# santi-pdp/segan_pytorch

Hardware: AMD Instinct MI355X
Metric: 16384-sample waveform chunks/sec (GAN step) (higher is better)
Workload: dtype f32

## Files before the change

segan_pytorch_amd/_lib.py:

```python
import ctypes
import os
import re
from ctypes import POINTER, Structure, c_char_p, c_double, c_float, c_int, c_int32, c_int64, c_size_t, c_void_p

_HERE = os.path.dirname(os.path.abspath(__file__))
LIB_PATH = os.environ.get('SEGAN_HIP_LIB') or os.path.join(_HERE, 'libsegan_hip.so')
HEADER_PATH = os.path.join(os.path.dirname(_HERE), 'include', 'segan_hip.h')
EXT_HEADER_PATH = os.path.join(os.path.dirname(_HERE), 'include', 'segan_dereverb.h')
PYIN_HEADER_PATH = os.path.join(os.path.dirname(_HERE), 'include', 'segan_pyin.h')
OMLSA_HEADER_PATH = os.path.join(os.path.dirname(_HERE), 'include', 'segan_omlsa.h')
RIR_HEADER_PATH = os.path.join(os.path.dirname(_HERE), 'include', 'segan_rir.h')


class SeganSrc(Structure):
    _fields_ = [('p0', c_void_p), ('p1', c_void_p), ('C0', c_int32), ('C1', c_int32),
                ('scale', c_void_p), ('shift', c_void_p), ('slope', c_void_p)]


_SCALARS = {'int': c_int, 'float': c_float, 'double': c_double, 'size_t': c_size_t,
            'int64_t': c_int64, 'long long': c_int64}


class _Defines(dict):

    def __init__(self, where):
        dict.__init__(self)
        self.where, self.unread = where, {}

    def __missing__(self, name):
        raise RuntimeError('{}: no integer `#define {}` ({})'.format(
            self.where, name, self.unread.get(name, 'not defined')))


def _ctype(text, decl, ret=False):
    tok = [w for w in re.findall(r'\w+|\S', text) if w != 'const']
    if not ret:
        if len(tok) < 2 or not re.match(r'[A-Za-z_]\w*$', tok[-1]):
            raise RuntimeError('unnamed or unreadable argument `{}` in `{}`'.format(text.strip(), decl))
        tok.pop()
    stars = tok.count('*')
    base = tok[:len(tok) - stars]
    if stars and base and '*' not in base:
        if not ret:
            return POINTER(SeganSrc) if tok == ['segan_src', '*'] else c_void_p
# ... 12 lines not shown
    seen = {}
    for name, val in re.findall(r'^[ \t]*#[ \t]*define[ \t]+(SEGAN_\w+)[ \t]+(\S.*?)[ \t]*$', text, flags=re.M):
        seen.setdefault(name, []).append(val)
    for name, vals in seen.items():
        if len(set(vals)) == 1 and re.match(r'-?(0[xX][0-9a-fA-F]+|[1-9]\d*|0)$', vals[0]):
            defines[name] = int(vals[0], 0)
        else:
            defines.unread[name] = ' / '.join('#define {} {}'.format(name, v) for v in vals)
    text = re.sub(r'^[ \t]*#.*$', '', text, flags=re.M)
    signatures = {}
    for m in re.finditer(r'[^;{}]*\bsegan_\w+\s*\([^;]*(;|$)', text):
        decl = ' '.join(m.group().split())
        d = re.match(r'([\w\s*]+?)\s*\b(segan_\w+)\s*\(([^()]*)\)\s*;$', decl)
        if not d or d.group(2) in signatures:
            raise RuntimeError('{}: cannot read the declaration `{}`'.format(where, decl))
        args = [] if d.group(3).strip() == 'void' else d.group(3).split(',')
        signatures[d.group(2)] = (_ctype(d.group(1), decl, ret=True), [_ctype(a, decl) for a in args])
    return signatures, defines


def _read_header_file(path=HEADER_PATH):
    if not os.path.exists(path):
        raise RuntimeError('segan_pytorch_amd: {} not found. The ctypes binding is read from the '
                           'header the library is built against.'.format(path))
    with open(path) as f:
        return read_header(f.read(), path)


SIGNATURES, DEFINES = _read_header_file()
EXT_SIGNATURES, EXT_DEFINES = _read_header_file(EXT_HEADER_PATH)
PYIN_SIGNATURES, PYIN_DEFINES = _read_header_file(PYIN_HEADER_PATH)
OMLSA_SIGNATURES, OMLSA_DEFINES = _read_header_file(OMLSA_HEADER_PATH)
RIR_SIGNATURES, RIR_DEFINES = _read_header_file(RIR_HEADER_PATH)

PAD_REFLECT = DEFINES['SEGAN_PAD_REFLECT']
PAD_ZERO = DEFINES['SEGAN_PAD_ZERO']
ACT_NONE = DEFINES['SEGAN_ACT_NONE']
ACT_TANH = DEFINES['SEGAN_ACT_TANH']
ABI_VERSION = DEFINES['SEGAN_ABI_VERSION']

_lib = None


def load():
    global _lib
    if _lib is not None:
        return _lib
    if not os.path.exists(LIB_PATH):
        raise RuntimeError(
            'segan_pytorch_amd: {} not found. Build it with `make` (or '
            '`python -c "import __graft_entry__ as g; g.build()"`) at the repo root. '
            'There is no non-HIP fallback.'.format(LIB_PATH))
    try:
        import torch
        if torch.cuda.is_available():
            torch.cuda.init()
    except ImportError:
        pass
    lib = ctypes.CDLL(LIB_PATH)
    for name, (res, args) in (list(SIGNATURES.items()) + list(EXT_SIGNATURES.items()) +
                              list(PYIN_SIGNATURES.items()) + list(OMLSA_SIGNATURES.items()) +
                              list(RIR_SIGNATURES.items())):
        fn = getattr(lib, name)
        fn.restype = res
        fn.argtypes = args
    ver = lib.segan_abi_version()
    if ver != ABI_VERSION:
        raise RuntimeError('libsegan_hip ABI {} != expected {}'.format(ver, ABI_VERSION))
    _lib = lib
    return lib


def check(rc, what=''):
    if rc != 0:
        msg = load().segan_last_error()
        raise RuntimeError('libsegan_hip {} failed ({}): {}'.format(
            what, rc, msg.decode() if msg else '?'))
```

segan_pytorch_amd/csrc/segan_conv.hip:

```cpp
#include "segan_conv_tile.h"


struct TileWork {
  int tile, c0, c1;
  bool partial;
  int piece;
};

struct TileIter {
  int tileA;
  long unit, unit_end;
  int first_tile;
  __device__ __forceinline__ void init(const CorrArgs& a, int nch) {
    tileA = blockIdx.x;
    unit = (long)blockIdx.x * a.sk_units;
    unit_end = min(unit + (long)a.sk_units, a.sk_total);
    first_tile = (int)(unit / nch);
  }
  __device__ __forceinline__ bool next(const CorrArgs& a, int nch, TileWork& w) {
    if (tileA < a.sk_nfull) {
      const int rd = tileA / (int)gridDim.x;
      const int left = a.sk_nfull - rd * (int)gridDim.x;
      w.tile = rd * (int)gridDim.x + xcd_remap(blockIdx.x, left < (int)gridDim.x ? left : (int)gridDim.x);
      w.c0 = 0; w.c1 = nch; w.partial = false; w.piece = 0;
      tileA += gridDim.x;
      return true;
    }
    if (unit < unit_end) {
      const int t = (int)(unit / nch);
      w.c0 = (int)(unit - (long)t * nch);
      w.c1 = min(nch, w.c0 + (int)(unit_end - unit));
      unit += w.c1 - w.c0;
      w.tile = a.sk_nfull + t;
// ... 890 lines not shown
  a.sk_ws_floats = scratch ? scratch_bytes / sizeof(float) : 0;
}

extern "C" size_t segan_bf16_scratch_bytes(int op, int B, int N, int M, int L, int K, int S, int pad,
                                           int planes) {
  if (!stride_ok(S) || B <= 0 || N <= 0 || M <= 0 || L <= 0 || L % S != 0 || planes < 1 || planes > 3)
    return 0;
  const int U = 32 / S, Ls = L / S;
  const size_t slabs = 256 + (size_t)1024 * 2 * 128 * 128 * sizeof(float);
  switch (op) {
    case 0: return slabs + segan_corr_bf2_scratch_bytes(B, N * S, Ls, U - 1, planes);
    case 3: return slabs + segan_corr_bf2_scratch_bytes(B, N * S, Ls, U - 1, planes);
    case 2: {
      int cmin = 1 << 30, cmax = 0;
      for (int r = 0; r < S; ++r) {
        const int c = (r + pad) / S;
        cmin = c < cmin ? c : cmin;
        cmax = c > cmax ? c : cmax;
      }
      return slabs + segan_corr_bf2_scratch_bytes(B, M, Ls, U - 1 + (cmax - cmin), planes);
    }
    case 1: {
      const int padR = K - S - pad > 0 ? K - S - pad : 0;
      return slabs + segan_corr_bf2_scratch_bytes(B, M, (L + pad + padR - 1) / S + 1, U - 1, planes);
    }
  }
  return 0;
}

extern "C" size_t segan_corr_scratch_bytes(void) {
  return (size_t)1024 * 2 * 128 * 128 * sizeof(float);
}

extern "C" int segan_conv1d_fwd(const segan_src* x, const void* wf, const float* bias, float* out,
                                int B, int N, int M, int L, int K, int S, int padL, int mode,
                                int roll, int precision, void* scratch, size_t scratch_bytes,
                                void* stream) {
  const int acc_block = precision == SEGAN_PREC_FP32_BLOCKED;
  if (acc_block) precision = SEGAN_PREC_FP32;
  SEGAN_REQUIRE(precision_ok(precision), "conv1d_fwd: precision must be 0, 1, 3 or 4");
  SEGAN_REQUIRE(stride_ok(S), "conv1d_fwd: stride %d not in {1,2,4}", S);
  SEGAN_REQUIRE(K >= 1 && K <= 32, "conv1d_fwd: kernel width %d not in [1,32]", K);
  SEGAN_REQUIRE(B > 0 && N > 0 && M > 0 && L > 0, "conv1d_fwd: bad sizes");
  SEGAN_REQUIRE(L % S == 0, "conv1d_fwd: length %d not divisible by stride %d", L, S);
  SEGAN_REQUIRE(wf && out, "conv1d_fwd: NULL pointer");
  SEGAN_REQUIRE(mode == SEGAN_PAD_REFLECT || mode == SEGAN_PAD_ZERO, "conv1d_fwd: bad pad mode");
  SEGAN_REQUIRE(mode != SEGAN_PAD_REFLECT || (padL < L && K - S - padL < L),
                "conv1d_fwd: reflect padding %d needs length > pad (L=%d)", padL, L);
  SEGAN_REQUIRE(roll > -L && roll < L, "conv1d_fwd: |roll| must be < L");
  if (int e = check_src(x, N, "conv1d_fwd")) return e;
  const int U = 32 / S;
  CorrArgs a = {};
  a.acc_block = acc_block;
  a.in = *x;
  a.wp = (const float*)wf;
  a.out0 = out; a.out1 = nullptr; a.bias = bias; a.halo = nullptr;
  a.B = B; a.Cv = N * S; a.Ktot = N * 32; a.RP = f_pitch(M); a.Rvalid = M;
  a.Tcols = L / S; a.Ctot = B * a.Tcols;
  a.Lin = L; a.padL = padL; a.mode = mode; a.roll = roll;
  a.win_start = 0; a.H = U - 1;
  a.NP = 1; a.Nout = 0;
  a.OC0 = M; a.OC1 = 0; a.Lout = a.Tcols; a.act = SEGAN_ACT_NONE;
  a.out0_elems = (size_t)B * M * a.Tcols;
  a.f_pair = f_pair(N, K); a.zphase = -1;
  if (precision) {
    CorrArgs a2 = a;
    const int e = segan_corr_bf2_f(a2, U, wf, precision, scratch, scratch_bytes, (hipStream_t)stream);
    return e;
  }
  if (N <= 2) return segan_launch_fsmall(a, M, N, S, (hipStream_t)stream);
  set_scratch(a, scratch, scratch_bytes);
  return launch_corr<true, false>(a, U, (hipStream_t)stream);
}

extern "C" int segan_deconv1d_dgrad(const float* dy, const void* wf, float* dx0, float* dx1, int B,
                                    int M, int M0, int N, int Ls, int K, int S, int pad,
                                    int precision, void* scratch, size_t scratch_bytes,
                                    void* stream) {
  const int acc_block = precision == SEGAN_PREC_FP32_BLOCKED;
  if (acc_block) precision = SEGAN_PREC_FP32;
  SEGAN_REQUIRE(precision_ok(precision), "deconv1d_dgrad: precision must be 0, 1, 3 or 4");
  SEGAN_REQUIRE(stride_ok(S), "deconv1d_dgrad: stride %d not in {1,2,4}", S);
  SEGAN_REQUIRE(K >= 1 && K <= 32, "deconv1d_dgrad: kernel width %d not in [1,32]", K);
  SEGAN_REQUIRE(B > 0 && N > 0 && M > 0 && Ls > 0, "deconv1d_dgrad: bad sizes");
  SEGAN_REQUIRE(M0 >= 0 && M0 <= M, "deconv1d_dgrad: split %d outside [0,%d]", M0, M);
  SEGAN_REQUIRE(dy && wf, "deconv1d_dgrad: NULL pointer");
  SEGAN_REQUIRE(dx0 || dx1, "deconv1d_dgrad: both destinations NULL");
  const int U = 32 / S;
  CorrArgs a = {};
  a.acc_block = acc_block;
  a.in.p0 = dy; a.in.p1 = nullptr; a.in.C0 = N; a.in.C1 = 0;
  a.in.scale = a.in.shift = a.in.slope = nullptr;
  a.wp = (const float*)wf;
  a.bias = nullptr; a.halo = nullptr;
  a.B = B; a.Cv = N * S; a.Ktot = N * 32; a.RP = f_pitch(M); a.Rvalid = M;
  a.Tcols = Ls; a.Ctot = B * Ls;
  a.Lin = S * Ls; a.padL = pad; a.mode = SEGAN_PAD_ZERO; a.roll = 0;
  a.win_start = 0; a.H = U - 1;
  a.NP = 1; a.Nout = 0;
  if (M0 == 0) { a.out0 = dx1; a.OC0 = M; a.out1 = nullptr; a.OC1 = 0; }
  else { a.out0 = dx0; a.OC0 = M0; a.out1 = dx1; a.OC1 = M - M0; }
  a.Lout = Ls; a.act = SEGAN_ACT_NONE;
  a.out0_elems = (size_t)B * a.OC0 * Ls;
  a.out1_elems = (size_t)B * a.OC1 * Ls;
  a.f_pair = f_pair(N, K); a.zphase = -1;
// ... 174 lines not shown
```

segan_pytorch_amd/csrc/segan_conv_edge.hip:

```cpp
#include "segan_conv_shared.h"

template <int S, int N, int PM, int KT>
__global__ __launch_bounds__(256) void tsmall_kernel(const CorrArgs a, const float* __restrict__ w,
                                                     int Krt, int M) {
  const int K = KT ? KT : Krt;
  constexpr int U = 32 / S;
  constexpr int MC = 16;
  constexpr int TW = 256 + U;
  __shared__ float xs[MC][TW + 1];
  const int tid = threadIdx.x;
  const int b = blockIdx.y;
  const int q0 = blockIdx.x * 256;
  const int q = q0 + tid;
  float acc[S][N];
#pragma unroll
  for (int r = 0; r < S; ++r)
#pragma unroll
    for (int n = 0; n < N; ++n) acc[r][n] = 0.0f;

  const int t0 = q0 + a.win_start + tid, t1 = t0 + 256;
  const bool ok0 = t0 >= 0 && t0 < a.Lin, ok1 = tid < U && t1 >= 0 && t1 < a.Lin;
  const int o0 = ok0 ? t0 : 0, o1 = ok1 ? t1 : 0;
  const int bo0 = b * a.in.C0 * a.Lin, bo1 = b * a.in.C1 * a.Lin;
  float pv0[MC], pv1[MC];
// ... 350 lines not shown
    float xv[N][32];
#pragma unroll
    for (int n = 0; n < N; ++n) {
      if (S == 4) {
#pragma unroll
        for (int i = 0; i < 8; ++i) {
          const f32x4 v = *reinterpret_cast<const f32x4*>(&xs[n][4 * tid + 4 * i]);
          xv[n][4 * i] = v[0]; xv[n][4 * i + 1] = v[1]; xv[n][4 * i + 2] = v[2]; xv[n][4 * i + 3] = v[3];
        }
      } else {
#pragma unroll
        for (int k = 0; k < 32; ++k) xv[n][k] = xs[n][S * tid + k];
      }
    }
    const int mcn = min(64, M - m0);
    for (int ml = 0; ml < mcn; ++ml) {
      float acc = a.bias ? a.bias[m0 + ml] : 0.0f;
#pragma unroll
      for (int n = 0; n < N; ++n) {
#pragma unroll
        for (int i = 0; i < 8; ++i) {
          const f32x4 wv = *reinterpret_cast<const f32x4*>(&ws[ml * WST + n * 32 + 4 * i]);
#pragma unroll
          for (int e = 0; e < 4; ++e) acc = fmaf(wv[e], xv[n][4 * i + e], acc);
        }
      }
      if (t < a.Lout) a.out0[((size_t)b * M + m0 + ml) * a.Lout + t] = acc;
    }
    __syncthreads();
  }
}


template <int S, int N, int RPT>
__global__ __launch_bounds__(256) void fsmall4_kernel(const CorrArgs a, const float* __restrict__ wq,
                                                      const float* __restrict__ bias, int M) {
  static_assert(S == 2 || S == 4, "fsmall4: strides 2 and 4");
  constexpr int Q = 4, U = 32 / S, MC = 8, CP = MC / 2;
  constexpr int XW = S * Q * 256 + 32;
  constexpr int XR = (S * (Q - 1) + 32 + 3) / 4 * 4;
  typedef float f32x2 __attribute__((ext_vector_type(2)));
  __shared__ __attribute__((aligned(16))) float xs[N][XW];
  const int tid = threadIdx.x;
  const int b = blockIdx.y;
  const int t0 = blockIdx.x * (Q * 256);
  fsmall_stage_window<S, N, XW>(a, b, t0, tid, xs);
  __syncthreads();
  const int t = t0 + Q * tid;
  f32x2 xv[N][XR / 2];
#pragma unroll
  for (int n = 0; n < N; ++n)
#pragma unroll
    for (int i = 0; i < XR / 4; ++i) {
      const f32x4 v = *reinterpret_cast<const f32x4*>(&xs[n][S * Q * tid + 4 * i]);
      xv[n][2 * i] = f32x2{v[0], v[1]};
      xv[n][2 * i + 1] = f32x2{v[2], v[3]};
    }
  const int RP = RPT ? RPT : a.RP;
  const bool vec = (a.Lout & 3) == 0 && t + Q <= a.Lout;
  typedef const __attribute__((address_space(4))) f32x2 cf2;
  for (int m0 = 0; m0 < M; m0 += MC) {
    f32x2 acc[CP][Q];
#pragma unroll
    for (int c = 0; c < CP; ++c) {
      const int ma = m0 + 2 * c < M ? m0 + 2 * c : M - 1, mb = m0 + 2 * c + 1 < M ? m0 + 2 * c + 1 : M - 1;
      const f32x2 bs = bias ? f32x2{bias[ma], bias[mb]} : f32x2{0.0f, 0.0f};
#pragma unroll
// ... 11 lines not shown
      }
    };
    auto fm = [&](const f32x2 (&w)[4][CP], int g, int e0, int e1) {
      const int n = g >> 3;
#pragma unroll
      for (int e = e0; e < e1; ++e)
#pragma unroll
        for (int c = 0; c < CP; ++c)
#pragma unroll
          for (int q = 0; q < Q; ++q) {
            const int j = S * q + 4 * (g & 7) + e;
            if (j & 1)
              asm("v_pk_fma_f32 %0, %1, %2, %0 op_sel:[0,1,0]"
                  : "+v"(acc[c][q]) : "s"(w[e][c]), "v"(xv[n][j >> 1]));
            else
              asm("v_pk_fma_f32 %0, %1, %2, %0 op_sel_hi:[1,0,1]"
                  : "+v"(acc[c][q]) : "s"(w[e][c]), "v"(xv[n][j >> 1]));
          }
    };
    ld(wa, 0);
#pragma unroll
    for (int g = 0; g < 8 * N; g += 2) {
      fm(wa, g, 0, 1);
      __builtin_amdgcn_sched_barrier(0);
      ld(wb, g + 1);
      __builtin_amdgcn_sched_barrier(0);
      fm(wa, g, 1, 4);
      fm(wb, g + 1, 0, 1);
      __builtin_amdgcn_sched_barrier(0);
      if (g + 2 < 8 * N) ld(wa, g + 2);
      __builtin_amdgcn_sched_barrier(0);
      fm(wb, g + 1, 1, 4);
    }
#pragma unroll
    for (int c = 0; c < MC; ++c) {
      if (m0 + c >= M) break;
      float* o = a.out0 + ((size_t)b * M + m0 + c) * a.Lout + t;
      if (vec) {
        const f32x4 ov = {acc[c / 2][0][c & 1], acc[c / 2][1][c & 1], acc[c / 2][2][c & 1], acc[c / 2][3][c & 1]};
        *reinterpret_cast<f32x4*>(o) = ov;
      } else {
#pragma unroll
        for (int q = 0; q < Q; ++q)
          if (t + q < a.Lout) o[q] = acc[c / 2][q][c & 1];
      }
    }
  }
}

int segan_launch_fsmall(CorrArgs& a, int M, int N, int S, hipStream_t st) {
  if (int e = segan_src_defaults(&a.in, st, "fsmall")) return e;
  if ((S == 4 || S == 2) && a.Lout >= 1024) {
    dim3 grid4(ceil_div(a.Lout, 1024), a.B);
#define FS4(SS, NN, RR) hipLaunchKernelGGL((fsmall4_kernel<SS, NN, RR>), grid4, dim3(256), 0, st, a, a.wp, a.bias, M)
    if (S == 4) {
      if (a.RP == 64) { if (N == 1) FS4(4, 1, 64); else FS4(4, 2, 64); }
      else { if (N == 1) FS4(4, 1, 0); else FS4(4, 2, 0); }
    } else {
      if (a.RP == 64) { if (N == 1) FS4(2, 1, 64); else FS4(2, 2, 64); }
      else { if (N == 1) FS4(2, 1, 0); else FS4(2, 2, 0); }
    }
#undef FS4
    return segan_check_launch("fsmall4_kernel");
  }
  dim3 grid(ceil_div(a.Lout, 256), a.B);
#define FS(SS, NN) hipLaunchKernelGGL((fsmall_kernel<SS, NN>), grid, dim3(256), 0, st, a, M)
  if (N == 1) { if (S == 4) FS(4, 1); else if (S == 2) FS(2, 1); else FS(1, 1); }
  else { if (S == 4) FS(4, 2); else if (S == 2) FS(2, 2); else FS(1, 2); }
#undef FS
  return segan_check_launch("fsmall_kernel");
}
```

segan_pytorch_amd/csrc/segan_conv_shared.h:

```cpp
#pragma once
#include "segan_common.h"
#include <stdlib.h>

#define KCH 64

struct ColTile {
  int col0, b0, t_first, len0;
};

__device__ __forceinline__ ColTile make_coltile(int col0, int Tcols, int NBcols) {
  ColTile t;
  t.col0 = col0;
  t.b0 = col0 / Tcols;
  t.t_first = col0 - t.b0 * Tcols;
  t.len0 = min(Tcols - t.t_first, NBcols);
  return t;
}

__device__ __forceinline__ void lds_pos_decode(const ColTile& ct, int j, int Tcols, int H, int& s,
                                               int& tau) {
  if (j < ct.len0 + H) {
    s = 0;
    tau = ct.t_first + j;
  } else {
// ... 11 lines not shown
  return x * q + (x < r ? x : r) + k;
}

struct CorrArgs {
  segan_src in;
  const float* wp;
  float* out0;
  float* out1;
  const float* bias;
  float* halo;
  int B, Cv, Ktot, RP, Rvalid;
  int Tcols, Ctot, ncoltiles;
  int Lin;
  int padL, mode, roll;
  int win_start, H, RLs;
  int rowshift[4];
  int NP, Nout;
  int OC0, OC1, Lout, act;
  int o_padL, o_roll, o_padR;
  int in_identity;
  int sk_nfull;
  int sk_units;
  long sk_total;
  int rt0;
  size_t out0_elems, out1_elems, halo_elems;
  float* sk_ws;
  size_t sk_ws_floats;
  int xf_mode;
  int acc_block;
  int RLv, nld;
  int f_pair;
  int zphase;
  int tile_order, nrt;
};



static inline int samples_per_tile(int Tcols, int NB) {
  if (Tcols >= NB) return (Tcols % NB == 0) ? 1 : 2;
  return (NB % Tcols == 0) ? NB / Tcols : (NB + Tcols - 2) / Tcols + 1;
}

static inline int t_np(int N, int S) { return round_up(N, 128 / S); }

struct WgradArgs {
  segan_src lo;
  segan_src hi;
  float* dw;
  int B, M, N, K, Ls, Lhi;
  int Cv;
  int padL, mode, roll;
  int Ctot;
  int cols_per_split;
  int H, RLw;
  int ls_magic;
  int per_magic;
  int bf_qc;
  int bf_cps;
  int Mp;
  int w2_cps, w2_nch;
  int w2_cpsample;
  int w2_spc;
  int w2_lsshift;
  int w2_pw, w2_nld;
  float* w2_slabs;
};
// ... 36 lines not shown
    int nb = 0;
    if (hipOccupancyMaxActiveBlocksPerMultiprocessor(&nb, reinterpret_cast<const void*>(kern), 256,
                                                     lds) != hipSuccess || nb < 1)
      nb = fallback;
    occ[d] = nb > 4 ? 4 : nb;
    occ_lds[d] = lds;
  }
  return occ[d];
}

static inline int f_pitch(int M) { return M <= 64 ? 64 : round_up(M, 128); }
static inline int f_rows(int N) { return round_up(N * 32, KCH); }
static inline int t_pitch(int N, int S) { return S * t_np(N, S); }
static inline int t_rows(int M, int S) { return round_up(M * (32 / S), KCH); }

static inline int f_pair(int N, int K) { return K == 31 && N > 2 && (N & 1) == 0; }
static inline int t_zphase(int K, int S, int pad_t) {
  return (K == 31 && S > 1) ? (((S - 1 - pad_t) % S) + S) % S : -1;
}

static inline bool stride_ok(int S) { return S == 1 || S == 2 || S == 4; }
static inline bool precision_ok(int p) { return p == 0 || p == 1 || p == 3; }
static inline int check_src(const segan_src* s, int C, const char* what) {
  SEGAN_REQUIRE(s != nullptr && s->p0 != nullptr, "%s: source is NULL", what);
  SEGAN_REQUIRE(s->C0 > 0 && s->C1 >= 0 && s->C0 + s->C1 == C,
                "%s: channel segments %d+%d != %d", what, s->C0, s->C1, C);
  SEGAN_REQUIRE(s->C1 == 0 || s->p1 != nullptr, "%s: second segment pointer is NULL", what);
  return SEGAN_OK;
}

int segan_launch_tsmall(CorrArgs& a, const float* w, int K, int M, int N, int S, int pad, hipStream_t st);
int segan_launch_fsmall(CorrArgs& a, int M, int N, int S, hipStream_t st);

void segan_note_corr_launch(int kind, unsigned grid, const CorrArgs& a, int ntiles);
int segan_corr_bf2_f(CorrArgs& a, int U, const void* wp3, int planes, void* scratch,
                     size_t scratch_bytes, hipStream_t st);
int segan_corr_bf2_t(CorrArgs& a, int U, const void* wp3, int planes, void* scratch,
                     size_t scratch_bytes, hipStream_t st);
size_t segan_corr_bf2_scratch_bytes(int B, int Cv, int Tcols, int H, int planes);
int segan_wgrad_bf2(WgradArgs& a, int U, int planes, void* scratch, size_t scratch_bytes, hipStream_t st);
void segan_note_wgrad_launch(int kind, int tiles, int nsplit, int chunks_per_split);
size_t segan_wgrad_bf2_scratch_bytes(int B, int M, int N, int Ls, int S, int planes);
```

segan_pytorch_amd/csrc/segan_pointwise.hip:

```cpp
#include "segan_common.h"

#define PW_THREADS 256

static int pw_nsplit(int B, int C, int L) {
  int ns = ceil_div(2048, C);
  if (ns > B) ns = B;
  long per = (long)B * L / ns;
  while (ns > 1 && per < 2048) {
    ns = (ns + 1) / 2;
    per = (long)B * L / ns;
  }
  return ns < 1 ? 1 : ns;
}

extern "C" int segan_bn_nsplit(int B, int C, int L) {
  if (B <= 0 || C <= 0 || L <= 0) return 0;
  return pw_nsplit(B, C, L);
}

template <int NV>
__device__ __forceinline__ void block_sum(float (&v)[NV], float* sm) {
  const int lane = threadIdx.x & 63, wave = threadIdx.x >> 6;
#pragma unroll
  for (int k = 0; k < NV; ++k) v[k] = warp_sum(v[k]);
  if (lane == 0)
#pragma unroll
    for (int k = 0; k < NV; ++k) sm[wave * NV + k] = v[k];
  __syncthreads();
  if (threadIdx.x == 0) {
#pragma unroll
    for (int k = 0; k < NV; ++k) {
      float s = 0.f;
      for (int w = 0; w < PW_THREADS / 64; ++w) s += sm[w * NV + k];
// ... 64 lines not shown
    }
  }
  float mean = 0.0f, m2 = 0.0f;
  if (n > 0.0f) {
    const float r = s1 / n;
    mean = K + r;
    m2 = fmaxf(s2 - s1 * r, 0.0f);
  }
#pragma unroll
  for (int o = 32; o > 0; o >>= 1) {
    const float nb2 = __shfl_down(n, o, 64), mb2 = __shfl_down(mean, o, 64), qb2 = __shfl_down(m2, o, 64);
    chan_combine(n, mean, m2, nb2, mb2, qb2);
  }
  const int lane = threadIdx.x & 63, wave = threadIdx.x >> 6;
  if (lane == 0) {
    sm[3 * wave] = n; sm[3 * wave + 1] = mean; sm[3 * wave + 2] = m2;
  }
  __syncthreads();
  if (threadIdx.x == 0) {
    for (int w = 1; w < PW_THREADS / 64; ++w) chan_combine(n, mean, m2, sm[3 * w], sm[3 * w + 1], sm[3 * w + 2]);
    float* w = ws + ((size_t)blockIdx.y * C + cr.c) * 3;
    w[0] = n;
    w[1] = mean;
    w[2] = m2;
  }
}

__device__ __forceinline__ void bn_affine(float gamma, float beta, float mean, float rstd,
                                          float& scale, float& shift) {
  scale = gamma * rstd;
  shift = fmaf(-mean, scale, beta);
}

__global__ void bn_final_kernel(const float* __restrict__ ws, const float* gamma, const float* beta,
                                float eps, float momentum, float* running_mean, float* running_var,
                                float* mean_o, float* rstd_o, float* scale_o, float* shift_o, int C,
                                int nsplit) {
  const int c = blockIdx.x * blockDim.x + threadIdx.x;
  if (c >= C) return;
  double n = 0.0, mean = 0.0, m2 = 0.0;
  for (int s = 0; s < nsplit; ++s) {
    const float* w = ws + ((size_t)s * C + c) * 3;
    const double nb = w[0], mb = w[1], qb = w[2];
    if (nb <= 0.0) continue;
    const double tot = n + nb;
    const double d = mb - mean;
    mean += d * nb / tot;
    m2 += qb + d * d * n * nb / tot;
    n = tot;
  }
  const double var = n > 0 ? m2 / n : 0.0;
  const float rstd = (float)(1.0 / sqrt(var + (double)eps));
  const float g = gamma ? gamma[c] : 1.0f;
  const float bt = beta ? beta[c] : 0.0f;
  float sc, sh;
  bn_affine(g, bt, (float)mean, rstd, sc, sh);
  if (mean_o) mean_o[c] = (float)mean;
  if (rstd_o) rstd_o[c] = rstd;
  if (scale_o) scale_o[c] = sc;
  if (shift_o) shift_o[c] = sh;
  if (running_mean) running_mean[c] = (1.0f - momentum) * running_mean[c] + momentum * (float)mean;
  if (running_var) {
    const double unb = n > 1 ? m2 / (n - 1.0) : var;
    running_var[c] = (1.0f - momentum) * running_var[c] + momentum * (float)unb;
  }
}

extern "C" int segan_bn_stats(const float* x, const float* gamma, const float* beta, float eps,
                              float momentum, float* running_mean, float* running_var, float* mean,
                              float* rstd, float* scale, float* shift, float* ws, int B, int C,
                              int L, void* stream) {
  SEGAN_REQUIRE(x && ws, "bn_stats: NULL pointer");
  SEGAN_REQUIRE(B > 0 && C > 0 && L > 0, "bn_stats: bad sizes");
  hipStream_t st = (hipStream_t)stream;
  const int ns = pw_nsplit(B, C, L);
  hipLaunchKernelGGL(bn_partial_kernel, dim3(C, ns), dim3(PW_THREADS), 0, st, x, ws, B, C, L, ns);
  hipLaunchKernelGGL(bn_final_kernel, dim3(ceil_div(C, 64)), dim3(64), 0, st, ws, gamma, beta, eps,
                     momentum, running_mean, running_var, mean, rstd, scale, shift, C, ns);
  return segan_check_launch("bn_stats");
}

extern "C" int segan_bn_partial(const float* x, float* ws, int B, int C, int L, void* stream) {
  SEGAN_REQUIRE(x && ws, "bn_partial: NULL pointer");
  SEGAN_REQUIRE(B > 0 && C > 0 && L > 0, "bn_partial: bad sizes");
  const int ns = pw_nsplit(B, C, L);
  hipLaunchKernelGGL(bn_partial_kernel, dim3(C, ns), dim3(PW_THREADS), 0, (hipStream_t)stream, x, ws,
                     B, C, L, ns);
  return segan_check_launch("bn_partial");
}

extern "C" int segan_bn_final(const float* ws, int nsplit_total, const float* gamma,
                              const float* beta, float eps, float momentum, float* running_mean,
                              float* running_var, float* mean, float* rstd, float* scale,
                              float* shift, int C, void* stream) {
  SEGAN_REQUIRE(ws && nsplit_total > 0 && C > 0, "bn_final: bad arguments");
  hipLaunchKernelGGL(bn_final_kernel, dim3(ceil_div(C, 64)), dim3(64), 0, (hipStream_t)stream, ws,
                     gamma, beta, eps, momentum, running_mean, running_var, mean, rstd, scale, shift,
                     C, nsplit_total);
// ... 721 lines not shown
```

segan_pytorch_amd/functional.py:

```python
import os

import torch

from . import ops
from .ops import ACT_NONE, ACT_TANH, PAD_REFLECT, PAD_ZERO, Src


def grad_buf(p):
    if p.grad is None:
        p.grad = torch.zeros_like(p, memory_format=torch.contiguous_format)
    elif not p.grad.is_contiguous():
        p.grad = p.grad.contiguous()
    return p.grad


def _gb(p, needed=True):
    if p is None or not needed or not p.requires_grad:
        return None
    return grad_buf(p)


def _bn_batch_stats(bn, training):
    return training or bn.running_mean is None or bn.running_var is None


def _bn_train_stats(c, bn, training=True):
    from . import distributed as sdist
    fn = sdist.bn_stats_sync if sdist.sync_bn_enabled() else ops.bn_stats
    track = training and bn.running_mean is not None and bn.running_var is not None
    momentum = 0.0
    if track:
        if bn.num_batches_tracked is not None:
            bn.num_batches_tracked += 1
        if bn.momentum is not None:
            momentum = bn.momentum
        else:
            momentum = 1.0 / float(bn.num_batches_tracked) if bn.num_batches_tracked is not None else 0.0
    return fn(c, bn.weight, bn.bias, bn.eps, momentum, bn.running_mean if track else None,
              bn.running_var if track else None)


def _bn_eval_affine(bn):
    rstd = torch.rsqrt(bn.running_var + bn.eps)
    gamma = bn.weight.detach() if bn.weight is not None else torch.ones_like(rstd)
    beta = bn.bias.detach() if bn.bias is not None else torch.zeros_like(rstd)
    scale = (gamma * rstd).contiguous()
    shift = (beta - bn.running_mean * scale).contiguous()
    return scale, shift, rstd.contiguous()


def _eval_bn_act_bwd(c, bn, scale, shift, rstd, dh, slope, dslope, y_tanh=None, dbias=None):
    if y_tanh is not None:
        g = ops.tanh_bwd(y_tanh, dh, dbias=_gb(bn.bias))
    else:
        v = ops.affine_prelu(c, scale, shift, None)
        g = ops.act_bwd(v, dh, slope=slope, dslope=dslope, dbias=_gb(bn.bias))
    if bn.weight is not None and bn.weight.requires_grad:
        xhat = ops.affine_prelu(c, rstd, (-bn.running_mean * rstd).contiguous(), None)
        grad_buf(bn.weight).add_((g * xhat).sum((0, 2)))
    dc = ops.affine_prelu(g, scale, None, None)
    if dbias is not None:
        ops.act_bwd(dc, dc, dbias=dbias)
    return dc


def _act_bwd_bn(a, dh, slope, bn, dslope, dgamma, dbeta, dbias):
    from . import distributed as sdist
    if sdist.sync_bn_enabled():
        return sdist.act_bwd_bn_sync(a, dh, slope, bn, dslope, dgamma, dbeta, dbias)
    return ops.act_bwd(a, dh, slope=slope, bn=bn, dslope=dslope, dgamma=dgamma, dbeta=dbeta,
                       dbias=dbias)

# ... 399 lines not shown
                if a_norm is None:
                    a_norm = ops.affine_prelu(a_enc[l], sc, sh, None)
                g = ops.act_bwd(a_norm, dh, dskip=dsk, slope=blk.act.weight, alpha=alpha_v,
                                dslope=_gb(blk.act.weight), dalpha=_gb(alpha_p, True))
                da = _act_bwd_bn(a_enc[l], g, None, bnsv, None, _gb(bnm.weight), _gb(bnm.bias),
                                 _gb(blk.conv.bias))
            padL = ops.conv_pad(K, S)[0]
            with _SideStream(da, src_enc[l]):
                if W.needs_grad(blk.conv):
                    gw = W.grad_target(blk.conv)
                    ops.wgrad(Src(da), src_enc[l], gw, K, S, padL, PAD_REFLECT)
                    W.finish(blk.conv, gw)
                _ready(blk, ready_extra)
            if l > 0:
                dh = ops.conv1d_dgrad(da, w, src_enc[l].L, S, pack=blk._pack)
            elif ctx.x_needs:
                dx = ops.conv1d_dgrad(da, w, src_enc[l].L, S, pack=blk._pack)
        _join_side(dy)
        ctx.state = None
        return (None, None, dx, None) + (None,) * (len(ctx.needs_input_grad) - 4)


class DiscriminatorFn(torch.autograd.Function):

    @staticmethod
    def forward(ctx, disc, rolls, x, x1, *params):
        x = x.contiguous()
        blocks = list(disc.enc_blocks)
        training = disc.training
        src = Src(x) if x1 is None else Src(x, x1.contiguous())
        cs, srcs, bns, xfs = [], [], [], []
        W = _Weights()
        for l, blk in enumerate(blocks):
            c = ops.conv1d_fwd(src, W.get(blk.conv), blk.conv.bias, blk.stride, roll=rolls[l],
                               pack=blk._pack)
            srcs.append(src)
            cs.append(c)
            if blk.norm is not None:
                bn = blk.norm
                if _bn_batch_stats(bn, training):
                    mean, rstd, scale, shift = _bn_train_stats(c, bn, training)
                    bns.append((mean, rstd, bn.weight, bn.bias))
                else:
                    scale, shift, _rstd = _bn_eval_affine(bn)
                    bns.append('eval')
                xfs.append((scale, shift))
                src = Src(c, scale=scale, shift=shift, slope=blk.act.weight)
            else:
                bns.append(None)
                xfs.append((None, None))
                src = Src(c, slope=blk.act.weight)
        h = ops.affine_prelu(cs[-1], xfs[-1][0], xfs[-1][1], blocks[-1].act.weight)
        B = h.shape[0]
        fc = disc.fc
        pt = disc.pool_type
        extra = {}
        if pt == 'none':
            hf = h.view(B, -1)
            y1 = ops.linear_fwd(hf, W.get(fc[0]))
            a1 = ops.bias_prelu_rows(y1, fc[0].bias, W.get(fc[1]))
            y2 = ops.linear_fwd(a1, W.get(fc[2]))
            a2 = ops.bias_prelu_rows(y2, fc[2].bias, W.get(fc[3]))
            y3 = ops.linear_fwd(a2, W.get(fc[4]))
            out = ops.bias_prelu_rows(y3, fc[4].bias, None)
            head = (hf, y1, a1, y2, a2, y3)
        else:
            if pt == 'conv':
                pc = ops.conv1d_fwd(Src(h), W.get(disc.pool_conv), disc.pool_conv.bias, 1,
                                    pad_mode=PAD_ZERO, padL=0, pack=disc._pool_pack)
                hp, idx = pc.view(B, -1), None
                extra['avg_conv_h'] = hp
            else:
                hp, idx = ops.pool_time_fwd(h, 'max' if pt == 'gmax' else 'avg')
            y3 = ops.linear_fwd(hp, W.get(fc))
# ... 317 lines not shown
```

segan_pytorch_amd/ops.py:

```python
import ctypes
import operator

import numpy as np
import torch

from . import _lib
from . import layout
from ._lib import ACT_NONE, ACT_TANH, PAD_REFLECT, PAD_ZERO, SeganSrc, check


import os as _os

_D = _lib.DEFINES
PREC_FP32, PREC_BF16, PREC_BF16X3 = _D['SEGAN_PREC_FP32'], _D['SEGAN_PREC_BF16'], _D['SEGAN_PREC_BF16X3']
_PREC_NAMES = {'fp32': PREC_FP32, 'bf16': PREC_BF16, 'bf16x3': PREC_BF16X3}
_precision = _PREC_NAMES[_os.environ.get('SEGAN_PRECISION', 'fp32')]
_EUNSUPPORTED = -3


_deterministic = _os.environ.get('SEGAN_DETERMINISTIC', '0') == '1'


def set_deterministic(on):
    global _deterministic
# ... 240 lines not shown
        buf = self._buf.get('g')
        if buf is None or buf.numel() * 4 != nbytes or buf.device != w.device:
            buf = torch.empty(nbytes // 4, device=w.device, dtype=torch.float32)
        check(lib.segan_pack_weights_g(_ptr(w), _ptr(buf), M, N, K, S, _stream()), 'pack_weights_g')
        self._buf['g'] = buf
        self._key['g'] = key
        return buf

    def t(self, w, S, pad_t):
        return self._get(w, S, pad_t, 't')

    def bf(self, w, S, pad_t, tform, planes):
        _chk(w, 'weight', 3)
        want = ('bf', tform, planes)
        key = (w.data_ptr(), w._version, _weights_epoch, getattr(w, '_segan_epoch', 0),
               tuple(w.shape), S, pad_t)
        if self._key.get(want) == key:
            return self._buf[want]
        lib = _lib.load()
        M, N, K = w.shape
        nbytes = lib.segan_packed_bf_bytes(M, N, S, tform, planes)
        if nbytes == 0:
            raise ValueError('unsupported geometry for bf16 packing')
        buf = self._buf.get(want)
        if buf is None or buf.numel() * 2 != nbytes or buf.device != w.device:
            buf = torch.empty(nbytes // 2, device=w.device, dtype=torch.bfloat16)
        check(lib.segan_pack_weights_bf(_ptr(w), _ptr(buf), M, N, K, S, tform, pad_t, planes,
                                        _stream()), 'pack_weights_bf')
        self._buf[want] = buf
        self._key[want] = key
        return buf


def conv1d_fwd(src, w, bias, S, roll=0, pad_mode=PAD_REFLECT, padL=None, pack=None):
    M, N, K = w.shape
    if src.C != N:
        raise ValueError('conv1d_fwd: input has {} channels, weight expects {}'.format(src.C, N))
    B, L = src.B, src.L
    if L % S != 0:
        raise ValueError('conv1d_fwd: length {} not divisible by stride {}'.format(L, S))
    if padL is None:
        padL = conv_pad(K, S)[0]
    out = torch.empty((B, M, L // S), device=w.device, dtype=torch.float32)
    cs = src.c_struct()
    pack = pack or WeightPack()
    lib = _lib.load()
    if _precision and pad_mode == PAD_REFLECT:
        keep, sp, sn = _bf_scratch(0, B, N, M, L, K, S, padL, w.device)
        rc = lib.segan_conv1d_fwd(ctypes.byref(cs), _ptr(pack.bf(w, S, 0, 0, _precision)),
                                  _ptr(bias), _ptr(out), B, N, M, L, K, S, padL, pad_mode, roll,
                                  _precision, sp, sn, _stream())
        if rc != _EUNSUPPORTED:
            check(rc, 'conv1d_fwd')
            return out
    check(lib.segan_conv1d_fwd(ctypes.byref(cs), _ptr(pack.f(w, S)), _ptr(bias), _ptr(out), B, N,
                               M, L, K, S, padL, pad_mode, roll, _fp32(), *_scratch(), _stream()),
          'conv1d_fwd')
    return out


def conv1d_dgrad(da, w, L, S, roll=0, padL=None, pack=None):
    _chk(da, 'da', 3)
    M, N, K = w.shape
    B = da.shape[0]
    if da.shape[1] != M or da.shape[2] * S != L:
        raise ValueError('conv1d_dgrad: da {} inconsistent with weight {} / L {}'.format(
            tuple(da.shape), tuple(w.shape), L))
    if padL is None:
        padL = conv_pad(K, S)[0]
    small = N <= 2
    _chk(w, 'weight', 3)
    pack = pack or WeightPack()
    if not small and not _precision and short_rows_ok(N, M, L, S):
        return conv1d_dgrad_short(da, w, L, S, roll=roll, padL=padL, pack=pack)
    dx = torch.empty((B, N, L), device=da.device, dtype=torch.float32)
    halo = torch.empty((B * N * max(K - 1, 1),), device=da.device, dtype=torch.float32)
    lib = _lib.load()
    if small:
        check(lib.segan_conv1d_dgrad(_ptr(da), None, _ptr(w.detach()), _ptr(dx), _ptr(halo), B, N,
# ... 2016 lines not shown
```

Baseline: 3556.

## Fuse batch-norm statistics into small-channel strided conv forward epilogue

Adds a BN-aware variant of the fsmall4 conv kernel that computes per-wave shifted sums and M2 for each output channel in registers and writes partial (n, mean, M2) triples to a workspace. A new wide reduction kernel then combines these partials in double precision to produce mean, rstd, scale, shift and running-stat updates. This avoids a separate pass that re-reads the conv output to compute batch statistics. It only applies to fp32, N<=2 input channels, stride 2 or 4 and long outputs, so in practice mainly the first discriminator layer; other layers fall back to the old path.

Result: no change. 3558, median of 2 (+0.1%).

```diff
diff --git a/include/segan_bnfuse.h b/include/segan_bnfuse.h
--- /dev/null
+++ b/include/segan_bnfuse.h
@@ -0,0 +1,26 @@
+#ifndef SEGAN_BNFUSE_H
+#define SEGAN_BNFUSE_H
+
+#include <stddef.h>
+#include "segan_hip.h"
+
+#ifdef __cplusplus
+extern "C" {
+#endif
+
+size_t segan_bnfuse_ws_floats(int B, int M, int L, int S);
+int segan_conv1d_fwd_bn(const segan_src* x, const void* wf, const float* bias, float* out, int B,
+                        int N, int M, int L, int K, int S, int padL, int mode, int roll,
+                        int precision, void* scratch, size_t scratch_bytes, const float* gamma,
+                        const float* beta, float eps, float momentum, float* running_mean,
+                        float* running_var, float* mean, float* rstd, float* scale, float* shift,
+                        float* ws, size_t ws_floats, void* stream);
+int segan_bn_final_wide(const float* ws, int nsplit_total, const float* gamma, const float* beta,
+                        float eps, float momentum, float* running_mean, float* running_var,
+                        float* mean, float* rstd, float* scale, float* shift, int C, void* stream);
+
+#ifdef __cplusplus
+}
+#endif
+
+#endif
diff --git a/segan_pytorch_amd/_lib.py b/segan_pytorch_amd/_lib.py
--- a/segan_pytorch_amd/_lib.py
+++ b/segan_pytorch_amd/_lib.py
@@ -10,6 +10,7 @@
 PYIN_HEADER_PATH = os.path.join(os.path.dirname(_HERE), 'include', 'segan_pyin.h')
 OMLSA_HEADER_PATH = os.path.join(os.path.dirname(_HERE), 'include', 'segan_omlsa.h')
 RIR_HEADER_PATH = os.path.join(os.path.dirname(_HERE), 'include', 'segan_rir.h')
+BNFUSE_HEADER_PATH = os.path.join(os.path.dirname(_HERE), 'include', 'segan_bnfuse.h')
 
 
 class SeganSrc(Structure):
@@ -88,6 +89,7 @@
 PYIN_SIGNATURES, PYIN_DEFINES = _read_header_file(PYIN_HEADER_PATH)
 OMLSA_SIGNATURES, OMLSA_DEFINES = _read_header_file(OMLSA_HEADER_PATH)
 RIR_SIGNATURES, RIR_DEFINES = _read_header_file(RIR_HEADER_PATH)
+BNFUSE_SIGNATURES, BNFUSE_DEFINES = _read_header_file(BNFUSE_HEADER_PATH)
 
 PAD_REFLECT = DEFINES['SEGAN_PAD_REFLECT']
 PAD_ZERO = DEFINES['SEGAN_PAD_ZERO']
@@ -116,7 +118,7 @@
     lib = ctypes.CDLL(LIB_PATH)
     for name, (res, args) in (list(SIGNATURES.items()) + list(EXT_SIGNATURES.items()) +
                               list(PYIN_SIGNATURES.items()) + list(OMLSA_SIGNATURES.items()) +
-                              list(RIR_SIGNATURES.items())):
+                              list(RIR_SIGNATURES.items()) + list(BNFUSE_SIGNATURES.items())):
         fn = getattr(lib, name)
         fn.restype = res
         fn.argtypes = args
diff --git a/segan_pytorch_amd/csrc/segan_conv.hip b/segan_pytorch_amd/csrc/segan_conv.hip
--- a/segan_pytorch_amd/csrc/segan_conv.hip
+++ b/segan_pytorch_amd/csrc/segan_conv.hip
@@ -1,4 +1,5 @@
 #include "segan_conv_tile.h"
+#include "../../include/segan_bnfuse.h"
 
 
 struct TileWork {
@@ -955,10 +956,18 @@
   return (size_t)1024 * 2 * 128 * 128 * sizeof(float);
 }
 
-extern "C" int segan_conv1d_fwd(const segan_src* x, const void* wf, const float* bias, float* out,
-                                int B, int N, int M, int L, int K, int S, int padL, int mode,
-                                int roll, int precision, void* scratch, size_t scratch_bytes,
-                                void* stream) {
+static size_t bnfuse_slots_bound(int B, int Ls) {
+  return (size_t)4 * B * (size_t)ceil_div(Ls, 1024);
+}
+extern "C" size_t segan_bnfuse_ws_floats(int B, int M, int L, int S) {
+  if (!stride_ok(S) || B <= 0 || M <= 0 || L <= 0 || L % S != 0 || (long)B * (L / S) >= (1L << 31)) return 0;
+  return bnfuse_slots_bound(B, L / S) * (size_t)M * 3;
+}
+
+static int conv1d_fwd_impl(const segan_src* x, const void* wf, const float* bias, float* out,
+                           int B, int N, int M, int L, int K, int S, int padL, int mode,
+                           int roll, int precision, void* scratch, size_t scratch_bytes,
+                           void* stream, float* bn_ws, size_t bn_ws_floats, int* bn_np) {
   const int acc_block = precision == SEGAN_PREC_FP32_BLOCKED;
   if (acc_block) precision = SEGAN_PREC_FP32;
   SEGAN_REQUIRE(precision_ok(precision), "conv1d_fwd: precision must be 0, 1, 3 or 4");
@@ -986,14 +995,53 @@
   a.OC0 = M; a.OC1 = 0; a.Lout = a.Tcols; a.act = SEGAN_ACT_NONE;
   a.out0_elems = (size_t)B * M * a.Tcols;
   a.f_pair = f_pair(N, K); a.zphase = -1;
+  if (bn_ws) {
+    if (precision || N > 2 || !((S == 4 || S == 2) && a.Lout >= 1024)) {
+      segan_set_error("conv1d_fwd_bn: geometry / precision not covered");
+      return SEGAN_EUNSUPPORTED;
+    }
+    SEGAN_REQUIRE(bn_ws_floats >= bnfuse_slots_bound(B, a.Tcols) * (size_t)M * 3,
+                  "conv1d_fwd_bn: workspace of %zu floats too small", bn_ws_floats);
+    a.bn_ws = bn_ws;
+  }
   if (precision) {
     CorrArgs a2 = a;
     const int e = segan_corr_bf2_f(a2, U, wf, precision, scratch, scratch_bytes, (hipStream_t)stream);
     return e;
   }
-  if (N <= 2) return segan_launch_fsmall(a, M, N, S, (hipStream_t)stream);
-  set_scratch(a, scratch, scratch_bytes);
-  return launch_corr<true, false>(a, U, (hipStream_t)stream);
+  int e;
+  if (N <= 2) {
+    e = segan_launch_fsmall(a, M, N, S, (hipStream_t)stream);
+  } else {
+    set_scratch(a, scratch, scratch_bytes);
+    e = launch_corr<true, false>(a, U, (hipStream_t)stream);
+  }
+  if (bn_np) *bn_np = a.bn_np;
+  return e;
+}
+
+extern "C" int segan_conv1d_fwd(const segan_src* x, const void* wf, const float* bias, float* out,
+                                int B, int N, int M, int L, int K, int S, int padL, int mode,
+                                int roll, int precision, void* scratch, size_t scratch_bytes,
+                                void* stream) {
+  return conv1d_fwd_impl(x, wf, bias, out, B, N, M, L, K, S, padL, mode, roll, precision, scratch,
+                         scratch_bytes, stream, nullptr, 0, nullptr);
+}
+
+extern "C" int segan_conv1d_fwd_bn(const segan_src* x, const void* wf, const float* bias, float* out,
+                                   int B, int N, int M, int L, int K, int S, int padL, int mode,
+                                   int roll, int precision, void* scratch, size_t scratch_bytes,
+                                   const float* gamma, const float* beta, float eps, float momentum,
+                                   float* running_mean, float* running_var, float* mean, float* rstd,
+                                   float* scale, float* shift, float* ws, size_t ws_floats,
+                                   void* stream) {
+  SEGAN_REQUIRE(ws != nullptr, "conv1d_fwd_bn: NULL workspace");
+  int np = 0;
+  if (int e = conv1d_fwd_impl(x, wf, bias, out, B, N, M, L, K, S, padL, mode, roll, precision, scratch,
+                              scratch_bytes, stream, ws, ws_floats, &np))
+    return e;
+  return segan_launch_bn_final_wide(ws, np, gamma, beta, eps, momentum, running_mean, running_var,
+                                    mean, rstd, scale, shift, M, (hipStream_t)stream);
 }
 
 extern "C" int segan_deconv1d_dgrad(const float* dy, const void* wf, float* dx0, float* dx1, int B,
diff --git a/segan_pytorch_amd/csrc/segan_conv_edge.hip b/segan_pytorch_amd/csrc/segan_conv_edge.hip
--- a/segan_pytorch_amd/csrc/segan_conv_edge.hip
+++ b/segan_pytorch_amd/csrc/segan_conv_edge.hip
@@ -406,7 +406,20 @@
 }
 
 
-template <int S, int N, int RPT>
+template <int HALF, int X>
+__device__ __forceinline__ void fsmall_bn_halve(float (&s1)[8], float (&s2)[8], float (&K)[8], int lane) {
+  const bool up = (lane & X) != 0;
+#pragma unroll
+  for (int r = 0; r < HALF; ++r) {
+    const float k1 = up ? s1[r + HALF] : s1[r], g1 = up ? s1[r] : s1[r + HALF];
+    const float k2 = up ? s2[r + HALF] : s2[r], g2 = up ? s2[r] : s2[r + HALF];
+    s1[r] = k1 + __shfl_xor(g1, X, 64);
+    s2[r] = k2 + __shfl_xor(g2, X, 64);
+    K[r] = up ? K[r + HALF] : K[r];
+  }
+}
+
+template <int S, int N, int RPT, bool BN = false>
 __global__ __launch_bounds__(256) void fsmall4_kernel(const CorrArgs a, const float* __restrict__ wq,
                                                       const float* __restrict__ bias, int M) {
   static_assert(S == 2 || S == 4, "fsmall4: strides 2 and 4");
@@ -484,6 +497,57 @@
       __builtin_amdgcn_sched_barrier(0);
       fm(wb, g + 1, 1, 4);
     }
+    if constexpr (BN) {
+      const int lane = tid & 63, wave = tid >> 6;
+      int nv = a.Lout - (t0 + Q * 64 * wave);
+      nv = nv < 0 ? 0 : (nv > Q * 64 ? Q * 64 : nv);
+      float r1[MC], r2[MC], rk[MC];
+#pragma unroll
+      for (int c = 0; c < CP; ++c) {
+        float k0 = acc[c][0][0], k1 = acc[c][0][1];
+        asm volatile("" : "+v"(k0));
+        asm volatile("" : "+v"(k1));
+        k0 = __builtin_bit_cast(float, __builtin_amdgcn_readfirstlane(__builtin_bit_cast(int, k0)));
+        k1 = __builtin_bit_cast(float, __builtin_amdgcn_readfirstlane(__builtin_bit_cast(int, k1)));
+        asm volatile("" : "+s"(k0));
+        asm volatile("" : "+s"(k1));
+        const f32x2 kk = {k0, k1};
+        f32x2 s1 = {0.0f, 0.0f}, s2 = {0.0f, 0.0f};
+#pragma unroll
+        for (int q = 0; q < Q; ++q) {
+          f32x2 d = acc[c][q] - kk;
+          if (t + q >= a.Lout) d = f32x2{0.0f, 0.0f};
+          s1 += d;
+          s2 += d * d;
+        }
+        r1[2 * c] = s1[0]; r1[2 * c + 1] = s1[1];
+        r2[2 * c] = s2[0]; r2[2 * c + 1] = s2[1];
+        rk[2 * c] = kk[0]; rk[2 * c + 1] = kk[1];
+      }
+      fsmall_bn_halve<4, 32>(r1, r2, rk, lane);
+      fsmall_bn_halve<2, 16>(r1, r2, rk, lane);
+      fsmall_bn_halve<1, 8>(r1, r2, rk, lane);
+#pragma unroll
+      for (int o = 4; o > 0; o >>= 1) {
+        r1[0] += __shfl_xor(r1[0], o, 64);
+        r2[0] += __shfl_xor(r2[0], o, 64);
+      }
+      const int m = m0 + ((lane >> 3) & 7);
+      if ((lane & 7) == 0 && m < M) {
+        const float n = (float)nv;
+        float mean = 0.0f, m2 = 0.0f;
+        if (nv > 0) {
+          const float r = r1[0] / n;
+          mean = rk[0] + r;
+          m2 = fmaxf(r2[0] - r1[0] * r, 0.0f);
+        }
+        const size_t slot = ((size_t)b * gridDim.x + blockIdx.x) * 4 + wave;
+        float* w = a.bn_ws + (slot * M + m) * 3;
+        w[0] = n;
+        w[1] = mean;
+        w[2] = m2;
+      }
+    }
 #pragma unroll
     for (int c = 0; c < MC; ++c) {
       if (m0 + c >= M) break;
@@ -504,7 +568,12 @@
   if (int e = segan_src_defaults(&a.in, st, "fsmall")) return e;
   if ((S == 4 || S == 2) && a.Lout >= 1024) {
     dim3 grid4(ceil_div(a.Lout, 1024), a.B);
-#define FS4(SS, NN, RR) hipLaunchKernelGGL((fsmall4_kernel<SS, NN, RR>), grid4, dim3(256), 0, st, a, a.wp, a.bias, M)
+    a.bn_np = (int)(grid4.x * grid4.y * 4);
+#define FS4(SS, NN, RR)                                                                                   \
+  do {                                                                                                    \
+    if (a.bn_ws) hipLaunchKernelGGL((fsmall4_kernel<SS, NN, RR, true>), grid4, dim3(256), 0, st, a, a.wp, a.bias, M); \
+    else hipLaunchKernelGGL((fsmall4_kernel<SS, NN, RR>), grid4, dim3(256), 0, st, a, a.wp, a.bias, M);   \
+  } while (0)
     if (S == 4) {
       if (a.RP == 64) { if (N == 1) FS4(4, 1, 64); else FS4(4, 2, 64); }
       else { if (N == 1) FS4(4, 1, 0); else FS4(4, 2, 0); }
diff --git a/segan_pytorch_amd/csrc/segan_conv_shared.h b/segan_pytorch_amd/csrc/segan_conv_shared.h
--- a/segan_pytorch_amd/csrc/segan_conv_shared.h
+++ b/segan_pytorch_amd/csrc/segan_conv_shared.h
@@ -67,6 +67,8 @@
   int f_pair;
   int zphase;
   int tile_order, nrt;
+  float* bn_ws;
+  int bn_np;
 };
 
 
@@ -169,6 +171,11 @@
 int segan_launch_tsmall(CorrArgs& a, const float* w, int K, int M, int N, int S, int pad, hipStream_t st);
 int segan_launch_fsmall(CorrArgs& a, int M, int N, int S, hipStream_t st);
 
+int segan_launch_bn_final_wide(const float* ws, int nsplit, const float* gamma, const float* beta,
+                               float eps, float momentum, float* running_mean, float* running_var,
+                               float* mean, float* rstd, float* scale, float* shift, int C,
+                               hipStream_t st);
+
 void segan_note_corr_launch(int kind, unsigned grid, const CorrArgs& a, int ntiles);
 int segan_corr_bf2_f(CorrArgs& a, int U, const void* wp3, int planes, void* scratch,
                      size_t scratch_bytes, hipStream_t st);
diff --git a/segan_pytorch_amd/csrc/segan_pointwise.hip b/segan_pytorch_amd/csrc/segan_pointwise.hip
--- a/segan_pytorch_amd/csrc/segan_pointwise.hip
+++ b/segan_pytorch_amd/csrc/segan_pointwise.hip
@@ -1,4 +1,5 @@
-#include "segan_common.h"
+#include "segan_conv_shared.h"
+#include "../../include/segan_bnfuse.h"
 
 #define PW_THREADS 256
 
@@ -129,6 +130,37 @@
   shift = fmaf(-mean, scale, beta);
 }
 
+__device__ __forceinline__ void bn_finish(int c, double n, double mean, double m2, const float* gamma,
+                                          const float* beta, float eps, float momentum,
+                                          float* running_mean, float* running_var, float* mean_o,
+                                          float* rstd_o, float* scale_o, float* shift_o) {
+  const double var = n > 0 ? m2 / n : 0.0;
+  const float rstd = (float)(1.0 / sqrt(var + (double)eps));
+  const float g = gamma ? gamma[c] : 1.0f;
+  const float bt = beta ? beta[c] : 0.0f;
+  float sc, sh;
+  bn_affine(g, bt, (float)mean, rstd, sc, sh);
+  if (mean_o) mean_o[c] = (float)mean;
+  if (rstd_o) rstd_o[c] = rstd;
+  if (scale_o) scale_o[c] = sc;
+  if (shift_o) shift_o[c] = sh;
+  if (running_mean) running_mean[c] = (1.0f - momentum) * running_mean[c] + momentum * (float)mean;
+  if (running_var) {
+    const double unb = n > 1 ? m2 / (n - 1.0) : var;
+    running_var[c] = (1.0f - momentum) * running_var[c] + momentum * (float)unb;
+  }
+}
+
+__device__ __forceinline__ void chan_combine_d(double& n, double& mean, double& m2, double nb,
+                                               double mb, double qb) {
+  if (nb <= 0.0) return;
+  const double tot = n + nb;
+  const double d = mb - mean;
+  mean += d * nb / tot;
+  m2 += qb + d * d * n * nb / tot;
+  n = tot;
+}
+
 __global__ void bn_final_kernel(const float* __restrict__ ws, const float* gamma, const float* beta,
                                 float eps, float momentum, float* running_mean, float* running_var,
                                 float* mean_o, float* rstd_o, float* scale_o, float* shift_o, int C,
@@ -146,21 +178,51 @@
     m2 += qb + d * d * n * nb / tot;
     n = tot;
   }
-  const double var = n > 0 ? m2 / n : 0.0;
-  const float rstd = (float)(1.0 / sqrt(var + (double)eps));
-  const float g = gamma ? gamma[c] : 1.0f;
-  const float bt = beta ? beta[c] : 0.0f;
-  float sc, sh;
-  bn_affine(g, bt, (float)mean, rstd, sc, sh);
-  if (mean_o) mean_o[c] = (float)mean;
-  if (rstd_o) rstd_o[c] = rstd;
-  if (scale_o) scale_o[c] = sc;
-  if (shift_o) shift_o[c] = sh;
-  if (running_mean) running_mean[c] = (1.0f - momentum) * running_mean[c] + momentum * (float)mean;
-  if (running_var) {
-    const double unb = n > 1 ? m2 / (n - 1.0) : var;
-    running_var[c] = (1.0f - momentum) * running_var[c] + momentum * (float)unb;
-  }
+  bn_finish(c, n, mean, m2, gamma, beta, eps, momentum, running_mean, running_var, mean_o, rstd_o,
+            scale_o, shift_o);
+}
+
+__global__ __launch_bounds__(PW_THREADS) void bn_final_wide_kernel(
+    const float* __restrict__ ws, const float* gamma, const float* beta, float eps, float momentum,
+    float* running_mean, float* running_var, float* mean_o, float* rstd_o, float* scale_o,
+    float* shift_o, int C, int nsplit) {
+  __shared__ double sm[3 * PW_THREADS];
+  const int c = blockIdx.x, t = threadIdx.x;
+  double n = 0.0, mean = 0.0, m2 = 0.0;
+  for (int s = t; s < nsplit; s += PW_THREADS) {
+    const float* w = ws + ((size_t)s * C + c) * 3;
+    chan_combine_d(n, mean, m2, w[0], w[1], w[2]);
+  }
+  sm[3 * t] = n; sm[3 * t + 1] = mean; sm[3 * t + 2] = m2;
+  __syncthreads();
+  for (int o = PW_THREADS / 2; o > 0; o >>= 1) {
+    if (t < o) {
+      chan_combine_d(n, mean, m2, sm[3 * (t + o)], sm[3 * (t + o) + 1], sm[3 * (t + o) + 2]);
+      sm[3 * t] = n; sm[3 * t + 1] = mean; sm[3 * t + 2] = m2;
+    }
+    __syncthreads();
+  }
+  if (t == 0)
+    bn_finish(c, n, mean, m2, gamma, beta, eps, momentum, running_mean, running_var, mean_o, rstd_o,
+              scale_o, shift_o);
+}
+
+int segan_launch_bn_final_wide(const float* ws, int nsplit, const float* gamma, const float* beta,
+                               float eps, float momentum, float* running_mean, float* running_var,
+                               float* mean, float* rstd, float* scale, float* shift, int C,
+                               hipStream_t st) {
+  hipLaunchKernelGGL(bn_final_wide_kernel, dim3(C), dim3(PW_THREADS), 0, st, ws, gamma, beta, eps,
+                     momentum, running_mean, running_var, mean, rstd, scale, shift, C, nsplit);
+  return segan_check_launch("bn_final_wide");
+}
+
+extern "C" int segan_bn_final_wide(const float* ws, int nsplit_total, const float* gamma,
+                                   const float* beta, float eps, float momentum, float* running_mean,
+                                   float* running_var, float* mean, float* rstd, float* scale,
+                                   float* shift, int C, void* stream) {
+  SEGAN_REQUIRE(ws && nsplit_total > 0 && C > 0, "bn_final_wide: bad arguments");
+  return segan_launch_bn_final_wide(ws, nsplit_total, gamma, beta, eps, momentum, running_mean,
+                                    running_var, mean, rstd, scale, shift, C, (hipStream_t)stream);
 }
 
 extern "C" int segan_bn_stats(const float* x, const float* gamma, const float* beta, float eps,
diff --git a/segan_pytorch_amd/functional.py b/segan_pytorch_amd/functional.py
--- a/segan_pytorch_amd/functional.py
+++ b/segan_pytorch_amd/functional.py
@@ -27,6 +27,11 @@
 def _bn_train_stats(c, bn, training=True):
     from . import distributed as sdist
     fn = sdist.bn_stats_sync if sdist.sync_bn_enabled() else ops.bn_stats
+    momentum, running_mean, running_var = _bn_track(bn, training)
+    return fn(c, bn.weight, bn.bias, bn.eps, momentum, running_mean, running_var)
+
+
+def _bn_track(bn, training):
     track = training and bn.running_mean is not None and bn.running_var is not None
     momentum = 0.0
     if track:
@@ -36,8 +41,18 @@
             momentum = bn.momentum
         else:
             momentum = 1.0 / float(bn.num_batches_tracked) if bn.num_batches_tracked is not None else 0.0
-    return fn(c, bn.weight, bn.bias, bn.eps, momentum, bn.running_mean if track else None,
-              bn.running_var if track else None)
+    return momentum, bn.running_mean if track else None, bn.running_var if track else None
+
+
+def _conv_bn_train(src, w, bias, S, bn, training, roll, pack):
+    from . import distributed as sdist
+    if sdist.sync_bn_enabled():
+        c = ops.conv1d_fwd(src, w, bias, S, roll=roll, pack=pack)
+        return (c,) + tuple(_bn_train_stats(c, bn, training))
+    momentum, running_mean, running_var = _bn_track(bn, training)
+    c, st = ops.conv1d_fwd_bn(src, w, bias, S, bn.weight, bn.bias, bn.eps, momentum, running_mean,
+                              running_var, roll=roll, pack=pack)
+    return (c,) + tuple(st)
 
 
 def _bn_eval_affine(bn):
@@ -503,14 +518,17 @@
         cs, srcs, bns, xfs = [], [], [], []
         W = _Weights()
         for l, blk in enumerate(blocks):
-            c = ops.conv1d_fwd(src, W.get(blk.conv), blk.conv.bias, blk.stride, roll=rolls[l],
-                               pack=blk._pack)
+            bn = blk.norm
+            if bn is not None and _bn_batch_stats(bn, training):
+                c, mean, rstd, scale, shift = _conv_bn_train(src, W.get(blk.conv), blk.conv.bias,
+                                                             blk.stride, bn, training, rolls[l], blk._pack)
+            else:
+                c = ops.conv1d_fwd(src, W.get(blk.conv), blk.conv.bias, blk.stride, roll=rolls[l],
+                                   pack=blk._pack)
             srcs.append(src)
             cs.append(c)
-            if blk.norm is not None:
-                bn = blk.norm
+            if bn is not None:
                 if _bn_batch_stats(bn, training):
-                    mean, rstd, scale, shift = _bn_train_stats(c, bn, training)
                     bns.append((mean, rstd, bn.weight, bn.bias))
                 else:
                     scale, shift, _rstd = _bn_eval_affine(bn)
diff --git a/segan_pytorch_amd/ops.py b/segan_pytorch_amd/ops.py
--- a/segan_pytorch_amd/ops.py
+++ b/segan_pytorch_amd/ops.py
@@ -296,6 +296,41 @@
         return buf
 
 
+_bn_fuse = _os.environ.get('SEGAN_BN_FUSE', '1') != '0'
+_pending_bn = None
+
+
+def set_bn_fuse(on):
+    global _bn_fuse
+    _bn_fuse = bool(on)
+
+
+def get_bn_fuse():
+    return _bn_fuse
+
+
+class _BnRequest(object):
+
+    def __init__(self, bn):
+        self.bn, self.result = bn, None
+
+
+def conv1d_fwd_bn(src, w, bias, S, gamma, beta, eps, momentum, running_mean, running_var, roll=0,
+                  pad_mode=PAD_REFLECT, padL=None, pack=None):
+    global _pending_bn
+    req = None
+    if _bn_fuse and not _precision and src.t0.is_cuda:
+        req = _BnRequest((gamma, beta, eps, momentum, running_mean, running_var))
+    _pending_bn = req
+    try:
+        out = conv1d_fwd(src, w, bias, S, roll=roll, pad_mode=pad_mode, padL=padL, pack=pack)
+    finally:
+        _pending_bn = None
+    if req is not None and req.result is not None:
+        return out, req.result
+    return out, bn_stats(out, gamma, beta, eps, momentum, running_mean, running_var)
+
+
 def conv1d_fwd(src, w, bias, S, roll=0, pad_mode=PAD_REFLECT, padL=None, pack=None):
     M, N, K = w.shape
     if src.C != N:
@@ -309,6 +344,23 @@
     cs = src.c_struct()
     pack = pack or WeightPack()
     lib = _lib.load()
+    global _pending_bn
+    req, _pending_bn = _pending_bn, None
+    if req is not None and not _precision and _fp32() == PREC_FP32:
+        C = M
+        stats = torch.empty((4, C), device=w.device, dtype=torch.float32)
+        nws = lib.segan_bnfuse_ws_floats(B, M, L, S)
+        ws = torch.empty((max(int(nws), 1),), device=w.device, dtype=torch.float32)
+        gamma, beta, eps, momentum, running_mean, running_var = req.bn
+        rc = lib.segan_conv1d_fwd_bn(ctypes.byref(cs), _ptr(pack.f(w, S)), _ptr(bias), _ptr(out), B, N,
+                                     M, L, K, S, padL, pad_mode, roll, PREC_FP32, *_scratch(),
+                                     _ptr(gamma), _ptr(beta), eps, momentum, _ptr(running_mean),
+                                     _ptr(running_var), _ptr(stats[0]), _ptr(stats[1]),
+                                     _ptr(stats[2]), _ptr(stats[3]), _ptr(ws), ws.numel(), _stream())
+        if rc != _EUNSUPPORTED:
+            check(rc, 'conv1d_fwd_bn')
+            req.result = (stats[0], stats[1], stats[2], stats[3])
+            return out
     if _precision and pad_mode == PAD_REFLECT:
         keep, sp, sn = _bf_scratch(0, B, N, M, L, K, S, padL, w.device)
         rc = lib.segan_conv1d_fwd(ctypes.byref(cs), _ptr(pack.bf(w, S, 0, 0, _precision)),
```
